# HKU-MedAI/WSI-HGNN

Hardware: AMD Instinct MI355X
Metric: edges/s fwd+bwd HEATNet4, 10k-node/6-rel synth graph, 1->8 MI355X (higher is better)
Workload: dtype f32 (fp16x3 emulation: 2-way fp16 split scaled per row (Y = XW^T, dX) or per column (dW), 3 products - bf16x6 for small launches; fp32-class error)

## Files before the change

### include/wsi_hgnn.h

```cpp
#ifndef WSI_HGNN_H
#define WSI_HGNN_H

#include <stdint.h>

#ifdef __cplusplus
extern "C" {
#endif

#define WSI_OK        0
#define WSI_EINVAL  (-22)
#define WSI_ENOSYS  (-38)
#define WSI_EFAULT  (-14)
#define WSI_ENOMEM  (-12)

#define WSI_ABI_VERSION 26

int         wsi_abi_version(void);
const char* wsi_last_error(void);

typedef struct wsi_context wsi_context_t;
int  wsi_context_create(wsi_context_t** out);
void wsi_context_destroy(wsi_context_t* ctx);

#define WSI_ATTN_XCD_CONTIGUOUS 1
// ... 198 lines not shown
int wsi_bag_slot_fill(const int64_t* bag_desc, int32_t num_bags, const int32_t* sel, float* rows, int64_t ld, int32_t feats,
                      int64_t num_rows, int32_t* row_seg, int32_t filler_seg,
                      const int32_t* small_src, int32_t* small_dst, int32_t small_words, void* stream);

typedef struct wsi_adam_tensor { float* p; const float* g; float* m; float* v; int64_t n; } wsi_adam_tensor_t;
int wsi_adam_step(const wsi_adam_tensor_t* tensors, int32_t count, double lr, double beta1, double beta2, double eps,
                  double weight_decay, int64_t step, void* stream);

#define WSI_OPTIM_SGD      0
#define WSI_OPTIM_ADAGRAD  1
#define WSI_OPTIM_ADADELTA 2
#define WSI_OPTIM_ADAM     3
#define WSI_OPTIM_FIRST    1
typedef struct wsi_optim_tensor {
    float* p; const float* g; float* s0; float* s1;
    float* step; int32_t* ticket; int64_t n; int32_t flags;
} wsi_optim_tensor_t;
typedef struct wsi_optim_hyper {
    double lr, weight_decay, momentum, dampening, nesterov, lr_decay, eps, rho, beta1, beta2, host_step;
} wsi_optim_hyper_t;
int wsi_optim_step(int32_t rule, const wsi_optim_tensor_t* tensors, int32_t count, const wsi_optim_hyper_t* hyper, void* stream);

int wsi_cross_entropy(const float* logits, const int64_t* labels, int32_t B, int32_t C, float* loss, float* dlogits, int32_t* bad_label, void* stream);

int wsi_segment_dot_diff(const float* g, int64_t ldg, const float* a, int64_t lda, const float* b, int64_t ldb,
                         int32_t D, const int32_t* chunk_row, int32_t num_chunks,
                         const int32_t* seg_chunk, int32_t num_segs,
                         float* partial, float* out, void* stream);

int wsi_gate_grad(const float* g, int64_t ldg, const float* a, int64_t lda, const float* b, int64_t ldb,
                  int32_t D, const int32_t* chunk_row, int32_t num_chunks, const int32_t* seg_chunk, int32_t num_segs,
                  const int32_t* seg_gate, const float* skip, int32_t n_gates, float* partial, float* g_skip, void* stream);

int wsi_pool_factors(const float* x, int64_t ldx, int32_t D, const float* w, int64_t ldw, int32_t T, int32_t H, int32_t Bg,
                     const int32_t* chunk_row, int32_t num_chunks, const int32_t* seg_chunk,
                     float* partial, float* hp, float* csum, float* x_mean, void* stream);
int wsi_pool_tmean(const float* tpart, int32_t T, int32_t S, int32_t D, int32_t H, const float* csum, const float* const* bv,
                   const float* scale, float* t_mean, void* stream);
int wsi_pool_bwd_prep(const float* g_pool, int32_t S, int32_t D, int32_t op, const float* counts, const float* z_mean, const float* h_mean,
                      const int32_t* seg_gate, const float* skip, int32_t n_gates, const int32_t* type_gate, int32_t T,
                      float* g_row, float* g_sum, float* g_skip, float* omg, void* stream);
int wsi_pool_bwd_bias(const float* gt_seg, int32_t T, int32_t S, int32_t D, int32_t H, const float* const* bv, const float* csum,
                      float* beta, float* gbv, void* stream);

int wsi_plan_assemble(const int64_t* desc, int32_t nsegs, int32_t total_blocks, void* stream);
int wsi_slot_fill(const int64_t* desc, int32_t nsegs, int32_t total_blocks, void* stream);

int wsi_layernorm_fwd(const float* x, int64_t ldx, int32_t n, int32_t D, float eps,
                      const float* gamma, const float* beta, const int32_t* row_param,
                      float* y, int64_t ldy, float* stats, void* stream);
int wsi_layernorm_bwd(const float* gy, int64_t ldgy, const float* x, int64_t ldx, int32_t n, int32_t D,
                      const float* gamma, const int32_t* row_param, const float* stats,
                      float* gx, int64_t ldgx, float* xhat_gy, int64_t ldp, void* stream);
int wsi_gelu_fwd(const float* x, float* y, int64_t n, void* stream);
int wsi_gelu_bwd(const float* x, const float* gy, float* gx, int64_t n, void* stream);
int wsi_spmm_sum(const float* x, int64_t ldx, int32_t n_out, int32_t D,
                 const int32_t* ptr, const int32_t* idx, const float* edge_w, const float* iscale, const float* oscale,
                 const float* bias, int32_t relu, const float* relu_ref, int64_t ldref,
                 float* out, int64_t ldo, void* stream);
int wsi_sddmm_dot(const float* g, int64_t ldg, const float* x, int64_t ldx, int32_t n, int32_t D,
                  const int32_t* rowptr, const int32_t* src, const float* iscale, const float* oscale,
                  const float* relu_ref, int64_t ldref, float* g_w, void* stream);

int wsi_row_sqnorm(const float* x, int64_t ldx, int32_t n, int32_t F, float* out, void* stream);
int wsi_knn_select(const float* dots, int64_t ldd, const float* sqnorm, int32_t row0, int32_t rows, int32_t N,
                   int32_t kc, int32_t* cand, void* stream);
// ... 166 lines not shown
```

### wsi-hgnn_amd/csrc/common.h

```cpp
#pragma once
#include <hip/hip_runtime.h>
#include <stdint.h>
#include <stdio.h>
#include <stdarg.h>
#include <stdlib.h>

#include "../../include/wsi_hgnn.h"

namespace wsi {

void set_error(const char* fmt, ...);

#ifdef WSI_ABLATE
inline const char* knob(const char* name) { return getenv(name); }
#else
constexpr const char* knob(const char*) { return nullptr; }
#endif

inline int check_launch(const char* what) {
    hipError_t e = hipGetLastError();
    if (e != hipSuccess) {
        set_error("%s: %s", what, hipGetErrorString(e));
        return WSI_EFAULT;
    }
    return WSI_OK;
}

template <int CTRL>
__device__ __forceinline__ float dpp_mov(float x) {
    return __int_as_float(__builtin_amdgcn_update_dpp(0, __float_as_int(x), CTRL, 0xf, 0xf, true));
}

template <int LPH>
__device__ __forceinline__ float group_sum(float x) {
    if (LPH >= 2) x += dpp_mov<0xB1>(x);
    if (LPH >= 4) x += dpp_mov<0x4E>(x);
    if (LPH >= 8) x += dpp_mov<0x141>(x);
    if (LPH >= 16) x += dpp_mov<0x140>(x);
    if (LPH >= 32) x += __shfl_xor(x, 16);
    if (LPH >= 64) x += __shfl_xor(x, 32);
    return x;
}

__device__ __forceinline__ float wave_sum(float x) { return group_sum<64>(x); }

template <int V>
__device__ __forceinline__ void load_vec(float (&r)[V], const float* __restrict__ p) {
    if constexpr (V % 4 == 0) {
#pragma unroll
        for (int i = 0; i < V / 4; ++i) {
            const float4 t = reinterpret_cast<const float4*>(p)[i];
            r[4 * i + 0] = t.x; r[4 * i + 1] = t.y; r[4 * i + 2] = t.z; r[4 * i + 3] = t.w;
        }
    } else if constexpr (V == 2) {
        const float2 t = *reinterpret_cast<const float2*>(p);
        r[0] = t.x; r[1] = t.y;
    } else {
#pragma unroll
        for (int i = 0; i < V; ++i) r[i] = p[i];
    }
}

template <int V>
__device__ __forceinline__ void store_vec(float* __restrict__ p, const float (&r)[V]) {
    if constexpr (V % 4 == 0) {
#pragma unroll
        for (int i = 0; i < V / 4; ++i)
            reinterpret_cast<float4*>(p)[i] = make_float4(r[4 * i], r[4 * i + 1], r[4 * i + 2], r[4 * i + 3]);
// ... 10 lines not shown
```

### wsi-hgnn_amd/csrc/heat_attn.hip

```cpp
#include "common.h"
#include <math.h>
#include <stdlib.h>
#include <mutex>
#include <type_traits>
#include <new>

namespace wsi {

struct AttnGraph {
    const int32_t* node_seg;
    const int32_t* rowptr;
    const int32_t* src;
    const float* sim;
    const int32_t* order;
    int32_t num_nodes;
    int32_t heavy_n;
    int32_t pass;
    int32_t heavy_deg;
    int32_t xcd;
    uint32_t* absmax;
    const float* score_in;
    const int32_t* gt_row;
};

// ... 318 lines not shown
                const float bj = beta[((int64_t)tau * S + (b * segs_per_type + gb)) * H + hh];
                gtab[(int64_t)ra * J + j] = acc_a[q] + bj;
                if (two) gtab[(int64_t)rbb * J + j] = acc_b[q] + bj;
            }
        }
    }
}

__global__ __launch_bounds__(256) void heat_attn_bwd_p1_flat_kernel(
    const int32_t* __restrict__ src, const int32_t* __restrict__ edge_seg, const int32_t* __restrict__ seg_dst,
    const int32_t* __restrict__ row_seg, int32_t segs_per_type, int32_t n_types, const float* __restrict__ inv_rd,
    const float* __restrict__ gtab, const float* __restrict__ lse, int64_t EH, int32_t H, const float* score_in, float* score_a, float* __restrict__ ga) {
    const int64_t o = (int64_t)blockIdx.x * 256 + threadIdx.x;
    if (o >= EH) return;
    const int64_t e = o / H;
    const int hh = (int)(o - e * H);
    const int s = edge_seg[e];
    const int w = seg_dst[s];
    const int b = row_seg[w] / segs_per_type;
    score_a[o] = expf(score_in[o] - lse[(int64_t)s * H + hh]);
    ga[o] = gtab[((int64_t)src[e] * n_types + b) * H + hh] * inv_rd[w];
}

__global__ __launch_bounds__(256) void heat_pool_coeff_kernel(
    const float* __restrict__ score, const float* __restrict__ lse, const int32_t* __restrict__ edge_seg,
    const int32_t* __restrict__ colptr, const int32_t* __restrict__ csc_eid, const int32_t* __restrict__ csc_dst,
    const float* __restrict__ inv_rd, const int32_t* __restrict__ row_seg, int32_t segs_per_type, int32_t n_types, int32_t H,
    int32_t num_src, float* __restrict__ ctab) {
    const int64_t idx = (int64_t)blockIdx.x * 256 + threadIdx.x;
    if (idx >= (int64_t)num_src * H) return;
    const int u = (int)(idx / H), h = (int)(idx - (int64_t)u * H);
    float cb[kPoolTypes];
#pragma unroll
    for (int b = 0; b < kPoolTypes; ++b) cb[b] = 0.f;
    const int j0 = colptr[u], j1 = colptr[u + 1];
    for (int j = j0; j < j1; ++j) {
        const int e = csc_eid[j], w = csc_dst[j];
        const float a = expf(score[(int64_t)e * H + h] - lse[(int64_t)edge_seg[e] * H + h]) * inv_rd[w];
        const int bin = row_seg[w] / segs_per_type;
#pragma unroll
        for (int b = 0; b < kPoolTypes; ++b) cb[b] += (bin == b) ? a : 0.f;
    }
#pragma unroll
    for (int b = 0; b < kPoolTypes; ++b)
        if (b < n_types) ctab[((int64_t)u * n_types + b) * H + h] = cb[b];
}

template <int V, int LPH, int U, bool COOP = false>
__global__ __launch_bounds__(kBlock) void heat_attn_bwd_p2_kernel(
    AttnTables tb, AttnGraph g, const float* __restrict__ e_weight, const float* __restrict__ e_bias,
    float inv_sqrt_dk, const float* __restrict__ a, const float* __restrict__ ga,
    float* __restrict__ gsc, float* __restrict__ gea, float* __restrict__ gq, int64_t ldgq) {
    constexpr int H = 64 / LPH;
    __shared__ float sm_acc[COOP ? kWavesPerBlock * 64 * V : 1];
    int lane;
    const int w = wave_uniform_node<COOP>(g, lane);
    if (w < 0) return;
    const int part = COOP ? (int)(threadIdx.x >> 6) : 0;
    constexpr int ESTEP = COOP ? kWavesPerBlock * U : U;
// ... 946 lines not shown
```

### wsi-hgnn_amd/csrc/loss.hip

```cpp
#include "common.h"
#include <math.h>

namespace wsi {

constexpr int64_t CE_IGNORE_INDEX = -100;
__global__ __launch_bounds__(256) void cross_entropy_kernel(const float* __restrict__ logits, const int64_t* __restrict__ labels, int B, int C,
                                                            float* __restrict__ loss, float* __restrict__ dlogits, int* __restrict__ bad) {
    __shared__ float part[256];
    __shared__ int cnt[256];
    __shared__ int any_bad;
    if (threadIdx.x == 0) any_bad = 0;
    int valid = 0;
    for (int b = threadIdx.x; b < B; b += 256) {
        const int64_t y = labels[b];
        valid += (y >= 0 && y < C) ? 1 : 0;
    }
    cnt[threadIdx.x] = valid;
    __syncthreads();
    for (int o = 128; o > 0; o >>= 1) {
        if ((int)threadIdx.x < o) cnt[threadIdx.x] += cnt[threadIdx.x + o];
        __syncthreads();
    }
    const int nvalid = cnt[0];
    const float invB = nvalid > 0 ? 1.f / (float)nvalid : 0.f;
    float acc = 0.f;
    for (int b = threadIdx.x; b < B; b += 256) {
        const float* row = logits + (int64_t)b * C;
        const int64_t y = labels[b];
        if (y < 0 || y >= C) {
            if (y != CE_IGNORE_INDEX) { any_bad = 1; if (bad) *bad = 1; }
            for (int c = 0; c < C; ++c) dlogits[(int64_t)b * C + c] = 0.f;
            continue;
        }
        float mx = -INFINITY;
// ... 1 lines not shown
        float den = 0.f;
        for (int c = 0; c < C; ++c) den += expf(row[c] - mx);
        acc += (logf(den) + mx) - row[y];
        const float inv = 1.f / den;
        for (int c = 0; c < C; ++c) dlogits[(int64_t)b * C + c] = (expf(row[c] - mx) * inv - (c == y ? 1.f : 0.f)) * invB;
    }
    part[threadIdx.x] = acc;
    __syncthreads();
    for (int o = 128; o > 0; o >>= 1) {
        if ((int)threadIdx.x < o) part[threadIdx.x] += part[threadIdx.x + o];
        __syncthreads();
    }
    if (threadIdx.x == 0) *loss = any_bad ? NAN : part[0] / (float)nvalid;
}

}

using namespace wsi;

extern "C" int wsi_cross_entropy(const float* logits, const int64_t* labels, int32_t B, int32_t C, float* loss, float* dlogits, int32_t* bad_label,
                                 void* stream) {
    if (B <= 0 || C <= 0 || (int64_t)B * C > 65536) { set_error("cross_entropy: unsupported shape %d x %d", B, C); return WSI_ENOSYS; }
    if (!logits || !labels || !loss || !dlogits) { set_error("cross_entropy: null pointer"); return WSI_EINVAL; }
    hipLaunchKernelGGL(cross_entropy_kernel, dim3(1), dim3(256), 0, (hipStream_t)stream, logits, labels, (int)B, (int)C, loss, dlogits, (int*)bad_label);
    return check_launch("cross_entropy");
}
```

### wsi-hgnn_amd/csrc/pooled.hip

```cpp
#include "common.h"
#include <math.h>

namespace wsi {

constexpr int POOL_MAX_TYPES = 16;
struct PtrList { const float* p[POOL_MAX_TYPES]; };

__global__ __launch_bounds__(256) void pool_tmean_kernel(const float* __restrict__ tpart, int tau0, int nt, int T, int S, int D, int H,
                                                         const float* __restrict__ csum, const PtrList bv, const float* __restrict__ scale,
                                                         int accumulate, int finish, float* __restrict__ t_mean) {
    const int s = blockIdx.x, c = blockIdx.y * 256 + threadIdx.x;
    if (c >= D) return;
    const int hh = c / (D / H);
    float acc = accumulate ? t_mean[(int64_t)s * D + c] : 0.f;
    for (int i = 0; i < nt; ++i) {
        const int tau = tau0 + i;
        acc += tpart[((int64_t)tau * S + s) * D + c];
        if (bv.p[i]) acc = fmaf(csum[((int64_t)tau * S + s) * H + hh], bv.p[i][c], acc);
    }
    if (finish && scale) acc *= scale[s];
    t_mean[(int64_t)s * D + c] = acc;
}

__global__ __launch_bounds__(256) void pool_bwd_prep_kernel(const float* __restrict__ g_pool, int S, int D, int mean, const float* __restrict__ counts,
// ... 4 lines not shown
                                                            float* __restrict__ omg) {
    extern __shared__ float dots[];
    const int lane = threadIdx.x & 63, wave = threadIdx.x >> 6;
    for (int s = wave; s < S; s += 4) {
        const float cnt = counts[s];
        const float fr = mean ? (cnt > 0.f ? 1.f / cnt : 0.f) : 1.f;
        const float fs = mean ? (cnt > 0.f ? 1.f : 0.f) : cnt;
        float acc = 0.f;
        for (int c = lane; c < D; c += 64) {
            const int64_t i = (int64_t)s * D + c;
            const float g = g_pool[i];
            const float gs = g * fs;
            g_row[i] = g * fr;
            g_sum[i] = gs;
            acc = fmaf(gs, z_mean[i] - h_mean[i], acc);
        }
        acc = wave_sum(acc);
        if (lane == 0) dots[s] = acc;
    }
    __syncthreads();
    for (int gt = threadIdx.x; gt < n_gates; gt += 256) {
        float acc = 0.f;
        for (int s = 0; s < S; ++s) acc += (seg_gate[s] == gt) ? dots[s] : 0.f;
        g_skip[gt] = acc * (1.f - 1.f / (1.f + expf(-skip[gt])));
    }
    for (int i = threadIdx.x; i < T; i += 256) {
        const int gt = type_gate[i];
        omg[i] = gt >= 0 ? 1.f - 1.f / (1.f + expf(-skip[gt])) : 1.f;
    }
}

__global__ __launch_bounds__(256) void pool_bwd_bias_kernel(const float* __restrict__ gt_seg, int tau0, int nt, int S, int D, int H, const PtrList bv,
                                                            const float* __restrict__ csum, float* __restrict__ beta, float* __restrict__ gbv) {
    const int dk = D / H;
    int blk = blockIdx.x;
    if (beta) {
        if (blk < nt * S) {
            const int i = blk / S, s = blk - i * S, tau = tau0 + i;
            const int lane = threadIdx.x & 63, wave = threadIdx.x >> 6;
            for (int hh = wave; hh < H; hh += 4) {
                float acc = 0.f;
                if (bv.p[i])
                    for (int c = lane; c < dk; c += 64) acc = fmaf(gt_seg[(int64_t)s * D + hh * dk + c], bv.p[i][hh * dk + c], acc);
                acc = wave_sum(acc);
                if (lane == 0) beta[((int64_t)tau * S + s) * H + hh] = acc;
            }
// ... 22 lines not shown
    hipStream_t st = (hipStream_t)stream;
    for (int t0 = 0; t0 < T; t0 += POOL_MAX_TYPES) {
        const int nt = (T - t0 < POOL_MAX_TYPES) ? T - t0 : POOL_MAX_TYPES;
        PtrList L;
        for (int i = 0; i < POOL_MAX_TYPES; ++i) L.p[i] = (i < nt) ? bv[t0 + i] : nullptr;
        hipLaunchKernelGGL(pool_tmean_kernel, dim3(S, (D + 255) / 256), dim3(256), 0, st, tpart, t0, nt, (int)T, (int)S, (int)D, (int)H, csum, L, scale,
                           t0 > 0 ? 1 : 0, t0 + nt >= T ? 1 : 0, t_mean);
    }
    return check_launch("pool_tmean");
}

extern "C" int wsi_pool_bwd_prep(const float* g_pool, int32_t S, int32_t D, int32_t op, const float* counts, const float* z_mean, const float* h_mean,
                                 const int32_t* seg_gate, const float* skip, int32_t n_gates, const int32_t* type_gate, int32_t T,
                                 float* g_row, float* g_sum, float* g_skip, float* omg, void* stream) {
    if (S <= 0 || S > 8192 || D <= 0 || n_gates <= 0 || T <= 0 || (op != WSI_RED_SUM && op != WSI_RED_MEAN)) { set_error("pool_bwd_prep: bad argument"); return WSI_EINVAL; }
    if (!g_pool || !counts || !z_mean || !h_mean || !seg_gate || !skip || !type_gate || !g_row || !g_sum || !g_skip || !omg) {
        set_error("pool_bwd_prep: null pointer"); return WSI_EINVAL;
    }
    hipLaunchKernelGGL(pool_bwd_prep_kernel, dim3(1), dim3(256), (size_t)S * sizeof(float), (hipStream_t)stream, g_pool, (int)S, (int)D,
                       op == WSI_RED_MEAN ? 1 : 0, counts, z_mean, h_mean, seg_gate, skip, (int)n_gates, type_gate, (int)T, g_row, g_sum, g_skip, omg);
    return check_launch("pool_bwd_prep");
}

extern "C" int wsi_pool_bwd_bias(const float* gt_seg, int32_t T, int32_t S, int32_t D, int32_t H, const float* const* bv, const float* csum,
                                 float* beta, float* gbv, void* stream) {
    if (T <= 0 || S <= 0 || D <= 0 || H <= 0 || D % H) { set_error("pool_bwd_bias: bad argument"); return WSI_EINVAL; }
    if (!gt_seg || (beta && !bv) || (gbv && !csum)) { set_error("pool_bwd_bias: null pointer"); return WSI_EINVAL; }
    if (!beta && !gbv) return WSI_OK;
    hipStream_t st = (hipStream_t)stream;
    const int tiles = (D + 255) / 256;
    for (int t0 = 0; t0 < T; t0 += POOL_MAX_TYPES) {
        const int nt = (T - t0 < POOL_MAX_TYPES) ? T - t0 : POOL_MAX_TYPES;
        PtrList L;
        for (int i = 0; i < POOL_MAX_TYPES; ++i) L.p[i] = (beta && i < nt) ? bv[t0 + i] : nullptr;
        const int blocks = (beta ? nt * S : 0) + (gbv ? nt * tiles : 0);
        hipLaunchKernelGGL(pool_bwd_bias_kernel, dim3(blocks), dim3(256), 0, st, gt_seg, t0, nt, (int)S, (int)D, (int)H, L, csum, beta, gbv);
    }
    return check_launch("pool_bwd_bias");
}
```

### wsi-hgnn_amd/csrc/segment.hip

```cpp
#include "common.h"
#include <math.h>

namespace wsi {

constexpr int SEG_THREADS = 256;

template <int OP>
__global__ __launch_bounds__(SEG_THREADS) void seg_stage1(const float* __restrict__ x, int64_t ldx, int32_t D, bool vec,
                                                           const int32_t* __restrict__ chunk_row,
                                                           float* __restrict__ partial, int32_t* __restrict__ partial_arg) {
    const int c = blockIdx.x;
    const int lane = threadIdx.x & 63, wave = threadIdx.x >> 6;
    const int col = blockIdx.y * 256 + lane * 4;
    const int r0 = chunk_row[c], r1 = chunk_row[c + 1];
    float a[4];
    int arg[4];
#pragma unroll
    for (int i = 0; i < 4; ++i) { a[i] = (OP == WSI_RED_MAX) ? -INFINITY : 0.f; arg[i] = -1; }
    if (col < D) {
        for (int r = r0 + wave; r < r1; r += 4) {
            const float* p = x + (int64_t)r * ldx + col;
            float v[4];
            if (vec && col + 3 < D) {
                const float4 t = *reinterpret_cast<const float4*>(p);
// ... 40 lines not shown
    const int col = blockIdx.y * SEG_THREADS + threadIdx.x;
    if (col >= D) return;
    const int c0 = seg_chunk[s], c1 = seg_chunk[s + 1];
    float acc = (OP == WSI_RED_MAX) ? -INFINITY : 0.f;
    int arg = -1;
    for (int c = c0; c < c1; ++c) {
        const float v = partial[(int64_t)c * D + col];
        if (OP == WSI_RED_MAX) {
            if (v > acc) { acc = v; arg = partial_arg[(int64_t)c * D + col]; }
        } else acc += v;
    }
    if (OP == WSI_RED_MEAN) {
        const int cnt = (c1 > c0) ? chunk_row[c1] - chunk_row[c0] : 0;
        acc = acc / (float)(cnt > 0 ? cnt : 1);
    }
    if (OP == WSI_RED_MAX) {
        if (arg < 0) acc = 0.f;
        argmax[(int64_t)s * D + col] = arg;
    }
    out[(int64_t)s * ldo + col] = acc;
}

constexpr int WSUM_J = 16;
__global__ __launch_bounds__(SEG_THREADS) void seg_wsum_stage1(const float* __restrict__ x, int64_t ldx, int32_t D, bool vec,
                                                                const float* __restrict__ w, int64_t ldw, int32_t JW, int32_t J,
                                                                const int32_t* __restrict__ chunk_row, float* __restrict__ partial,
                                                                float* __restrict__ wpartial) {
    const int c = blockIdx.x;
    const int lane = threadIdx.x & 63;
    const int wave = __builtin_amdgcn_readfirstlane((int)(threadIdx.x >> 6));
    const int col = blockIdx.y * 256 + lane * 4;
    const int jb = blockIdx.z * WSUM_J;
    const int nj = min(WSUM_J, J - jb);
    const int r0 = chunk_row[c], r1 = chunk_row[c + 1];
    float a[WSUM_J][4];
    float ws[WSUM_J];
#pragma unroll
    for (int j = 0; j < WSUM_J; ++j) {
        ws[j] = 0.f;
#pragma unroll
        for (int i = 0; i < 4; ++i) a[j][i] = 0.f;
    }
    if (col < D) {
        for (int r = r0 + wave; r < r1; r += 4) {
            const float* p = x + (int64_t)r * ldx + col;
            float v[4];
            if (vec && col + 3 < D) {
                const float4 t = *reinterpret_cast<const float4*>(p);
                v[0] = t.x; v[1] = t.y; v[2] = t.z; v[3] = t.w;
            } else {
#pragma unroll
                for (int i = 0; i < 4; ++i) v[i] = (col + i < D) ? p[i] : 0.f;
            }
            const float* wr = w + (int64_t)r * ldw + jb;
#pragma unroll
            for (int j = 0; j < WSUM_J; ++j) {
                const float wj = (jb + j < JW) ? wr[j] : ((j < nj) ? 1.f : 0.f);
                ws[j] += wj;
#pragma unroll
                for (int i = 0; i < 4; ++i) a[j][i] = fmaf(wj, v[i], a[j][i]);
            }
        }
    }
    if (wpartial && blockIdx.y == 0) {
        __shared__ float shw[4][WSUM_J];
        if (lane == 0) {
#pragma unroll
// ... 136 lines not shown

__global__ __launch_bounds__(256) void gate_grad_stage2(const float* __restrict__ partial, int32_t ncoltiles, const int32_t* __restrict__ seg_chunk,
                                                        int32_t num_segs, const int32_t* __restrict__ seg_gate, const float* __restrict__ skip,
                                                        int32_t n_gates, float* __restrict__ g_skip) {
    extern __shared__ float dots[];
    const int lane = threadIdx.x & 63, wave = threadIdx.x >> 6;
    for (int s = wave; s < num_segs; s += 4) {
        const int64_t p0 = (int64_t)seg_chunk[s] * ncoltiles, p1 = (int64_t)seg_chunk[s + 1] * ncoltiles;
        float acc = 0.f;
        for (int64_t i = p0 + lane; i < p1; i += 64) acc += partial[i];
        acc = wave_sum(acc);
        if (lane == 0) dots[s] = acc;
    }
    __syncthreads();
    for (int gt = threadIdx.x; gt < n_gates; gt += 256) {
        float acc = 0.f;
        for (int s = 0; s < num_segs; ++s) acc += (seg_gate[s] == gt) ? dots[s] : 0.f;
        g_skip[gt] = acc * (1.f - 1.f / (1.f + expf(-skip[gt])));
    }
}

static inline bool vec_ok(const void* p, int64_t ld) { return ((reinterpret_cast<uintptr_t>(p) & 15) == 0) && (ld % 4 == 0); }

}

using namespace wsi;

extern "C" int wsi_segment_reduce_fwd(const float* x, int64_t ldx, int32_t D, int32_t op,
                                      const int32_t* chunk_row, int32_t num_chunks,
                                      const int32_t* seg_chunk, int32_t num_segs,
                                      float* partial, float* out, int64_t ldo, int32_t* argmax, void* stream) {
    if (D <= 0 || num_chunks < 0 || num_segs < 0 || op < 0 || op > 2) { set_error("segment_reduce_fwd: bad argument"); return WSI_EINVAL; }
    if (num_segs == 0) return WSI_OK;
    if (!chunk_row || !seg_chunk || !out || (num_chunks > 0 && (!x || !partial))) { set_error("segment_reduce_fwd: null pointer"); return WSI_EINVAL; }
    if (op == WSI_RED_MAX && !argmax) { set_error("segment_reduce_fwd: max needs argmax"); return WSI_EINVAL; }
    hipStream_t st = (hipStream_t)stream;
    const bool vec = vec_ok(x, ldx);
    int32_t* parg = reinterpret_cast<int32_t*>(partial + (int64_t)num_chunks * D);
    const dim3 g1(num_chunks, (D + 255) / 256), g2(num_segs, (D + SEG_THREADS - 1) / SEG_THREADS);
    if (op == WSI_RED_SUM) {
        if (num_chunks) hipLaunchKernelGGL(seg_stage1<WSI_RED_SUM>, g1, dim3(SEG_THREADS), 0, st, x, ldx, D, vec, chunk_row, partial, (int32_t*)nullptr);
        hipLaunchKernelGGL(seg_stage2<WSI_RED_SUM>, g2, dim3(SEG_THREADS), 0, st, (const float*)partial, (const int32_t*)nullptr, D, chunk_row, seg_chunk, out, ldo, (int32_t*)nullptr);
    } else if (op == WSI_RED_MEAN) {
        if (num_chunks) hipLaunchKernelGGL(seg_stage1<WSI_RED_SUM>, g1, dim3(SEG_THREADS), 0, st, x, ldx, D, vec, chunk_row, partial, (int32_t*)nullptr);
        hipLaunchKernelGGL(seg_stage2<WSI_RED_MEAN>, g2, dim3(SEG_THREADS), 0, st, (const float*)partial, (const int32_t*)nullptr, D, chunk_row, seg_chunk, out, ldo, (int32_t*)nullptr);
    } else {
// ... 27 lines not shown
                                    float* partial, float* out, void* stream) {
    if (D <= 0 || num_chunks < 0 || num_segs < 0) { set_error("segment_dot_diff: bad argument"); return WSI_EINVAL; }
    if (num_segs == 0) return WSI_OK;
    if (!chunk_row || !seg_chunk || !out || (num_chunks > 0 && (!g || !a || !b || !partial))) { set_error("segment_dot_diff: null pointer"); return WSI_EINVAL; }
    hipStream_t st = (hipStream_t)stream;
    const int nct = (D + 255) / 256;
    const bool vec = vec_ok(g, ldg) && vec_ok(a, lda) && vec_ok(b, ldb);
    if (num_chunks) hipLaunchKernelGGL(seg_dot_stage1, dim3(num_chunks, nct), dim3(SEG_THREADS), 0, st, g, ldg, a, lda, b, ldb, D, vec, chunk_row, partial);
    hipLaunchKernelGGL(seg_dot_stage2, dim3(num_segs), dim3(64), 0, st, (const float*)partial, nct, seg_chunk, out);
    return check_launch("segment_dot_diff");
}

extern "C" int wsi_segment_weighted_sums(const float* x, int64_t ldx, int32_t D, const float* w, int64_t ldw, int32_t J,
                                         const int32_t* chunk_row, int32_t num_chunks, const int32_t* seg_chunk, int32_t num_segs,
                                         float* partial, float* out, void* stream) {
    if (D <= 0 || J <= 0 || J > 1024 || num_chunks < 0 || num_segs < 0) { set_error("segment_weighted_sums: bad argument"); return WSI_EINVAL; }
    if (num_segs == 0) return WSI_OK;
    if (!chunk_row || !seg_chunk || !out || (num_chunks > 0 && (!x || !w || !partial))) { set_error("segment_weighted_sums: null pointer"); return WSI_EINVAL; }
    if ((int64_t)J * D > INT32_MAX) { set_error("segment_weighted_sums: J * D too large"); return WSI_EINVAL; }
    hipStream_t st = (hipStream_t)stream;
    const bool vec = vec_ok(x, ldx);
    const int32_t JD = J * D;
    const dim3 g1(num_chunks, (D + 255) / 256, (J + WSUM_J - 1) / WSUM_J), g2(num_segs, (JD + SEG_THREADS - 1) / SEG_THREADS);
    if (num_chunks) hipLaunchKernelGGL(seg_wsum_stage1, g1, dim3(SEG_THREADS), 0, st, x, ldx, D, vec, w, ldw, J, J, chunk_row, partial, (float*)nullptr);
    hipLaunchKernelGGL(seg_stage2<WSI_RED_SUM>, g2, dim3(SEG_THREADS), 0, st, (const float*)partial, (const int32_t*)nullptr, JD, chunk_row, seg_chunk,
                       out, (int64_t)JD, (int32_t*)nullptr);
    return check_launch("segment_weighted_sums");
}

extern "C" int wsi_pool_factors(const float* x, int64_t ldx, int32_t D, const float* w, int64_t ldw, int32_t T, int32_t H, int32_t Bg,
                                const int32_t* chunk_row, int32_t num_chunks, const int32_t* seg_chunk,
                                float* partial, float* hp, float* csum, float* x_mean, void* stream) {
    if (D <= 0 || T <= 0 || H <= 0 || Bg <= 0 || num_chunks < 0 || (int64_t)T * H > 1024) { set_error("pool_factors: bad argument"); return WSI_EINVAL; }
    if (!chunk_row || !seg_chunk || !hp || !csum || (num_chunks > 0 && (!x || !w || !partial))) { set_error("pool_factors: null pointer"); return WSI_EINVAL; }
    const int32_t J = T * H, JT = J + (x_mean ? 1 : 0);
    if ((int64_t)JT * D > INT32_MAX) { set_error("pool_factors: T * H * D too large"); return WSI_EINVAL; }
    hipStream_t st = (hipStream_t)stream;
    float* wpartial = partial + (int64_t)num_chunks * JT * D;
    const dim3 g1(num_chunks, (D + 255) / 256, (JT + WSUM_J - 1) / WSUM_J);
    const dim3 g2(T * Bg, (uint32_t)(((int64_t)JT * D + SEG_THREADS - 1) / SEG_THREADS) + 1);
    if (num_chunks) hipLaunchKernelGGL(seg_wsum_stage1, g1, dim3(SEG_THREADS), 0, st, x, ldx, D, vec_ok(x, ldx), w, ldw, J, JT, chunk_row, partial, wpartial);
    hipLaunchKernelGGL(pool_factors_stage2, g2, dim3(SEG_THREADS), 0, st, (const float*)partial, (const float*)wpartial, D, T, H, Bg, JT, chunk_row, seg_chunk,
                       hp, csum, x_mean);
    return check_launch("pool_factors");
}

extern "C" int wsi_gate_grad(const float* g, int64_t ldg, const float* a, int64_t lda, const float* b, int64_t ldb,
                             int32_t D, const int32_t* chunk_row, int32_t num_chunks, const int32_t* seg_chunk, int32_t num_segs,
                             const int32_t* seg_gate, const float* skip, int32_t n_gates, float* partial, float* g_skip, void* stream) {
    if (D <= 0 || num_chunks < 0 || num_segs < 0 || n_gates <= 0 || num_segs > 8192) { set_error("gate_grad: bad argument"); return WSI_EINVAL; }
    if (!chunk_row || !seg_chunk || !seg_gate || !skip || !g_skip || (num_chunks > 0 && (!g || !a || !b || !partial))) { set_error("gate_grad: null pointer"); return WSI_EINVAL; }
    hipStream_t st = (hipStream_t)stream;
    const int nct = (D + 255) / 256;
    const bool vec = vec_ok(g, ldg) && vec_ok(a, lda) && vec_ok(b, ldb);
    if (num_chunks) hipLaunchKernelGGL(seg_dot_stage1, dim3(num_chunks, nct), dim3(SEG_THREADS), 0, st, g, ldg, a, lda, b, ldb, D, vec, chunk_row, partial);
    hipLaunchKernelGGL(gate_grad_stage2, dim3(1), dim3(256), (size_t)(num_segs > 0 ? num_segs : 1) * sizeof(float), st, (const float*)partial, nct, seg_chunk,
                       num_segs, seg_gate, skip, n_gates, g_skip);
    return check_launch("gate_grad");
}
```

### wsi-hgnn_amd/ops.py

```python
from __future__ import annotations

import array
import ctypes
import contextlib
from typing import List, Optional, Sequence, Tuple

import torch

from . import _native as N
from .graph import GraphPlan, SegmentTable, host_to_device



_TIMING = {"on": False, "records": []}


def enable_kernel_timing(on: bool) -> None:
    _TIMING["on"] = bool(on)
    _TIMING["records"] = []


class _Timed:
    def __init__(self, name: str, flops: float = 0.0, mfma_flops: float = 0.0):
        self.name, self.flops, self.mfma_flops = name, flops, mfma_flops
# ... 379 lines not shown
            N.check(lib.wsi_gemm_grouped(op, epilogue, prec, arr, len(chunk), N.ptr(ws), ws_bytes, N.stream()), "wsi_gemm_grouped")
    return wrote


_GROUP_FIELDS = [f[0] for f in N.GemmGroup._fields_]
_GROUP_INDEX = {name: i for i, name in enumerate(_GROUP_FIELDS)}
_GROUP_DEFAULT = tuple(1.0 if name == "drop_scale" else (None if N.GemmGroup._fields_[i][1] is ctypes.c_void_p else 0) for i, name in enumerate(_GROUP_FIELDS))


def _group_array(chunk):
    index, default = _GROUP_INDEX, _GROUP_DEFAULT
    rows = []
    for g in chunk:
        vals = list(default)
        for k, v in g.items():
            i = index.get(k)
            if i is not None:
                vals[i] = v
        rows.append(N.GemmGroup(*vals))
    return (N.GemmGroup * len(rows))(*rows)


_SMALL_PAIR = {"enabled": True}


def _gemm_small_pair(dx_groups: Sequence[dict], dx_epilogue: int, dw_groups: Sequence[dict], dw_epilogue: int, device) -> bool:
    dx_groups = [g for g in dx_groups if g["M"] > 0 and g["N"] > 0]
    dw_groups = [g for g in dw_groups if g["M"] > 0 and g["N"] > 0]
    if (not _SMALL_PAIR["enabled"] or not dx_groups or not dw_groups or len(dx_groups) + len(dw_groups) > 16
            or any(g["M"] > 32 or g.get("c_absmax") or g.get("b_chunk") for g in dx_groups) or any(g["K"] > 32 or g.get("c_absmax") for g in dw_groups)):
        return False
    flops = sum(2.0 * g["M"] * g["N"] * g["K"] for g in list(dx_groups) + list(dw_groups))
    with _Timed("gemm", flops, flops), _Timed("gemm_small_pair", flops, flops):
        N.check(N.load().wsi_gemm_small_pair(_group_array(dx_groups), len(dx_groups), dx_epilogue, _group_array(dw_groups), len(dw_groups), dw_epilogue,
                                             N.stream()), "wsi_gemm_small_pair")
    return True


_BACKGROUND = {"enabled": True, "min_flop": 3.0e10, "queued": [], "pending": [], "armed": False, "blocked": False,
               "launches": 0, "task": -1, "written": set()}


def set_background_weight_gradients(on: bool) -> None:
    _BACKGROUND["enabled"] = bool(on)


# ... 1083 lines not shown
        ctx.save_for_backward(h, kqv, t, out, score, lse, skip, ew, eb, sim_csr, *(() if (drop_mask is None or counter is not None) else (drop_mask,)), *params)
        return out

    @staticmethod
    def backward(ctx, g_out):
        lib = N.load()
        hctx, H, T = ctx.hctx, ctx.H, ctx.T
        bc = None
        if ctx.pool is not None:
            h, kqv, t_mean, h_mean, z_mean, score, lse, skip, ew, eb, sim_csr, *params = ctx.saved_tensors
            fwd_factors = None
            if ctx.no_v:
                fwd_factors, params = params[:3], params[3:]
            t = out = None
            prp, pop = ctx.pool
            n_rows, D_ = h.shape
            pre = None
            segs_p = prp.segments_of(hctx.rows)
            if prp.num_segs <= 8192 and segs_p is not None:
                seg_gate, type_gate = _gate_tables(hctx, skip, segs_p, prp.num_segs)
                g_pool = g_out.contiguous()
                g_row, g_sum = torch.empty_like(g_pool), torch.empty_like(g_pool)
                pre = (torch.empty_like(skip), torch.empty(T, dtype=torch.float32, device=h.device))
                N.check(lib.wsi_pool_bwd_prep(N.ptr(g_pool), prp.num_segs, D_, pop, N.ptr(prp.counts()), N.ptr(z_mean), N.ptr(h_mean), N.ptr(seg_gate),
                                              N.ptr(skip), skip.shape[0], N.ptr(type_gate), T, N.ptr(g_row), N.ptr(g_sum), N.ptr(pre[0]), N.ptr(pre[1]),
                                              N.stream()), "wsi_pool_bwd_prep")
                bc = SegmentBroadcast.from_parts(prp, g_row, g_sum, z_mean)
            else:
                bc = SegmentBroadcast.from_pooled_gradient(g_out.contiguous(), prp, pop, z_mean)
            collapse = ctx.no_v or _value_collapse_applies(hctx, prp, n_rows, D_, H)
            if collapse:
                g_out = None
            else:
                g_out = torch.empty((n_rows, D_), dtype=torch.float32, device=h.device)
                N.check(lib.wsi_segment_reduce_bwd(N.ptr(bc.g_row), D_, D_, N.WSI_RED_SUM, N.ptr(prp.chunk_row), N.ptr(prp.chunk_seg),
                                                   prp.num_chunks, N.ptr(prp.seg_chunk), prp.num_segs, None,
                                                   N.ptr(g_out), D_, N.stream()), "wsi_segment_reduce_bwd")
        else:
            h, kqv, t, out, score, lse, skip, ew, eb, sim_csr, *params = ctx.saved_tensors
            t_mean = h_mean = None
            collapse = False
            fwd_factors = None
            pre = None
            g_out = g_out.contiguous()
        g_y = g_out
        if ctx.has_mask and getattr(ctx, "counter", None) is not None:
            g_y = dropout_apply(g_out, ctx.counter)
        elif ctx.has_mask:
            g_y = g_out * params[0]
# ... 233 lines not shown
                grads[8 * tau + 6] = gbv[tau]
                for hh in range(H):
                    wgroups.append(dict(A=N.ptr(gt_seg, hh * dk * 4), lda=D, B=N.ptr(hp, (hh * T + tau) * D * 4), ldb=H * T * D,
                                        C=N.ptr(gw, hh * dk * D * 4), ldc=D, M=dk, N=D, K=S))
            _gemm(N.WSI_GEMM_TN, 0, wgroups, dev)
        if gh_max is not None and chunked:
            attach_row_scales(g_h, gh_max)
        if gh_cols is not None and gh_wrote and chunked:
            attach_col_stats(g_h, gh_cols)
        if early_gate is not None:
            torch.cuda.current_stream(dev).wait_event(early_gate[1])
        return (g_h, None, None, g_skip, g_e[0:1].view(1, 1), g_e[1:2], None, None, None, *grads)


def heat_layer_fused(h, hctx, H, skip, e_weight, e_bias, params, drop_mask=None, pool=None, background_dw=False):
    if pool is not None:
        pool = (pool[0], {"sum": N.WSI_RED_SUM, "mean": N.WSI_RED_MEAN}[pool[1]])
    return _HeatLayerFused.apply(h, hctx, H, skip, e_weight, e_bias, drop_mask, pool, background_dw, *params)


class _CrossEntropy(torch.autograd.Function):

    @staticmethod
    def forward(ctx, logits, labels, bad):
        N.require_cuda(logits, labels)
        logits = logits.contiguous()
        labels = labels.contiguous()
        if labels.dtype != torch.int64 or logits.dim() != 2 or labels.shape != logits.shape[:1]:
            raise ValueError("cross_entropy: logits [B, C] fp32 and int64 labels [B]")
        B, C = logits.shape
        out = torch.empty(1 + B * C, dtype=torch.float32, device=logits.device)
        N.check(N.load().wsi_cross_entropy(N.ptr(logits), N.ptr(labels), B, C, N.ptr(out), N.ptr(out, 4), N.ptr(bad), N.stream()), "wsi_cross_entropy")
        ctx.save_for_backward(out)
        ctx.shape = (B, C)
        return out[0]

    @staticmethod
    def backward(ctx, g):
        (out,) = ctx.saved_tensors
        return out[1:].view(ctx.shape) * g, None, None


def cross_entropy(logits: torch.Tensor, labels: torch.Tensor) -> torch.Tensor:
    bad = torch.zeros(1, dtype=torch.int32, device=logits.device)
    loss = _CrossEntropy.apply(logits, labels, bad)
    loss._wsi_bad_label = bad
    return loss


class _RelationAttention(torch.autograd.Function):

    @staticmethod
    def forward(ctx, q, kv, e_weight, e_bias, plan: GraphPlan, sim_csr, D: int, H: int):
        N.require_cuda(q, kv)
        lib = N.load()
        q = q.contiguous()
        kv = kv.contiguous()
        n, E, S = plan.num_nodes, plan.num_edges, plan.num_segs
        dev = q.device
        t = torch.empty((n, D), dtype=torch.float32, device=dev)
        score = torch.empty((max(E, 1), H), dtype=torch.float32, device=dev)
        lse = torch.empty((max(S, 1), H), dtype=torch.float32, device=dev)
        ew, eb = e_weight.reshape(-1), e_bias.reshape(-1)
        with _Timed("heat_attn"):
            N.check(lib.wsi_heat_attn_fwd(
                N.ptr(q), q.stride(0), N.ptr(kv, 0), kv.stride(0), N.ptr(kv, D * 4), kv.stride(0), n, D, H,
                N.ptr(plan.node_seg), N.ptr(plan.rowptr), N.ptr(plan.src), N.ptr(sim_csr), N.ptr(plan.order_dst), plan.num_heavy, _attn_flags(plan),
                N.ptr(ew), N.ptr(eb), N.ptr(t), D, N.ptr(score), N.ptr(lse), None, N.context(), N.stream()), "wsi_heat_attn_fwd")
# ... 1226 lines not shown
```

Before: 111.1 million.

## Spread pool backward prep across blocks, batch gathers, and drop CE zero-fill

```diff
diff --git a/include/wsi_hgnn.h b/include/wsi_hgnn.h
--- a/include/wsi_hgnn.h
+++ b/include/wsi_hgnn.h
@@ -244,6 +244,7 @@
 int wsi_optim_step(int32_t rule, const wsi_optim_tensor_t* tensors, int32_t count, const wsi_optim_hyper_t* hyper, void* stream);
 
 int wsi_cross_entropy(const float* logits, const int64_t* labels, int32_t B, int32_t C, float* loss, float* dlogits, int32_t* bad_label, void* stream);
+int wsi_cross_entropy_self(const float* logits, const int64_t* labels, int32_t B, int32_t C, float* loss, float* dlogits, int32_t* bad_label, void* stream);
 
 int wsi_segment_dot_diff(const float* g, int64_t ldg, const float* a, int64_t lda, const float* b, int64_t ldb,
                          int32_t D, const int32_t* chunk_row, int32_t num_chunks,
@@ -264,6 +265,9 @@
                       float* g_row, float* g_sum, float* g_skip, float* omg, void* stream);
 int wsi_pool_bwd_bias(const float* gt_seg, int32_t T, int32_t S, int32_t D, int32_t H, const float* const* bv, const float* csum,
                       float* beta, float* gbv, void* stream);
+int wsi_pool_bwd_prep_spread(const float* g_pool, int32_t S, int32_t D, int32_t op, const float* counts, const float* z_mean, const float* h_mean,
+                             const int32_t* seg_gate, const float* skip, int32_t n_gates, const int32_t* type_gate, int32_t T,
+                             float* g_row, float* g_sum, float* g_skip, float* omg, float* dots, int32_t* ticket, void* stream);
 
 int wsi_plan_assemble(const int64_t* desc, int32_t nsegs, int32_t total_blocks, void* stream);
 int wsi_slot_fill(const int64_t* desc, int32_t nsegs, int32_t total_blocks, void* stream);
diff --git a/wsi-hgnn_amd/csrc/common.h b/wsi-hgnn_amd/csrc/common.h
--- a/wsi-hgnn_amd/csrc/common.h
+++ b/wsi-hgnn_amd/csrc/common.h
@@ -44,6 +44,24 @@
 
 __device__ __forceinline__ float wave_sum(float x) { return group_sum<64>(x); }
 
+__device__ __forceinline__ void publish(float* p, float v) { __hip_atomic_store(p, v, __ATOMIC_RELAXED, __HIP_MEMORY_SCOPE_AGENT); }
+
+__device__ __forceinline__ bool arrive_last(int32_t* ticket, int blocks, int* flag) {
+    asm volatile("s_waitcnt vmcnt(0)" ::: "memory");
+    __syncthreads();
+    if (threadIdx.x == 0) {
+        const int last = __hip_atomic_fetch_add(ticket, 1, __ATOMIC_RELAXED, __HIP_MEMORY_SCOPE_AGENT) == blocks - 1;
+        if (last) {
+            __hip_atomic_exchange(ticket, 0, __ATOMIC_RELAXED, __HIP_MEMORY_SCOPE_AGENT);
+            __builtin_amdgcn_fence(__ATOMIC_ACQUIRE, "agent");
+            asm volatile("s_waitcnt vmcnt(0)" ::: "memory");
+        }
+        *flag = last;
+    }
+    __syncthreads();
+    return *flag != 0;
+}
+
 template <int V>
 __device__ __forceinline__ void load_vec(float (&r)[V], const float* __restrict__ p) {
     if constexpr (V % 4 == 0) {
diff --git a/wsi-hgnn_amd/csrc/heat_attn.hip b/wsi-hgnn_amd/csrc/heat_attn.hip
--- a/wsi-hgnn_amd/csrc/heat_attn.hip
+++ b/wsi-hgnn_amd/csrc/heat_attn.hip
@@ -364,6 +364,28 @@
     ga[o] = gtab[((int64_t)src[e] * n_types + b) * H + hh] * inv_rd[w];
 }
 
+template <int NB>
+__device__ __forceinline__ void pool_coeff_edges(int j, int h, int H, int segs_per_type, const float* __restrict__ score, const float* __restrict__ lse,
+                                                 const int32_t* __restrict__ edge_seg, const int32_t* __restrict__ csc_eid,
+                                                 const int32_t* __restrict__ csc_dst, const float* __restrict__ inv_rd,
+                                                 const int32_t* __restrict__ row_seg, float (&cb)[kPoolTypes]) {
+    int e[NB], w[NB], sg[NB], rs[NB];
+    float sc[NB], ls[NB], ir[NB];
+#pragma unroll
+    for (int i = 0; i < NB; ++i) { e[i] = csc_eid[j + i]; w[i] = csc_dst[j + i]; }
+#pragma unroll
+    for (int i = 0; i < NB; ++i) { sg[i] = edge_seg[e[i]]; sc[i] = score[(int64_t)e[i] * H + h]; ir[i] = inv_rd[w[i]]; rs[i] = row_seg[w[i]]; }
+#pragma unroll
+    for (int i = 0; i < NB; ++i) ls[i] = lse[(int64_t)sg[i] * H + h];
+#pragma unroll
+    for (int i = 0; i < NB; ++i) {
+        const float a = expf(sc[i] - ls[i]) * ir[i];
+        const int bin = rs[i] / segs_per_type;
+#pragma unroll
+        for (int b = 0; b < kPoolTypes; ++b) cb[b] += (bin == b) ? a : 0.f;
+    }
+}
+
 __global__ __launch_bounds__(256) void heat_pool_coeff_kernel(
     const float* __restrict__ score, const float* __restrict__ lse, const int32_t* __restrict__ edge_seg,
     const int32_t* __restrict__ colptr, const int32_t* __restrict__ csc_eid, const int32_t* __restrict__ csc_dst,
@@ -376,7 +398,10 @@
 #pragma unroll
     for (int b = 0; b < kPoolTypes; ++b) cb[b] = 0.f;
     const int j0 = colptr[u], j1 = colptr[u + 1];
-    for (int j = j0; j < j1; ++j) {
+    int j = j0;
+    for (; j + 8 <= j1; j += 8) pool_coeff_edges<8>(j, h, H, segs_per_type, score, lse, edge_seg, csc_eid, csc_dst, inv_rd, row_seg, cb);
+    for (; j + 4 <= j1; j += 4) pool_coeff_edges<4>(j, h, H, segs_per_type, score, lse, edge_seg, csc_eid, csc_dst, inv_rd, row_seg, cb);
+    for (; j < j1; ++j) {
         const int e = csc_eid[j], w = csc_dst[j];
         const float a = expf(score[(int64_t)e * H + h] - lse[(int64_t)edge_seg[e] * H + h]) * inv_rd[w];
         const int bin = row_seg[w] / segs_per_type;
diff --git a/wsi-hgnn_amd/csrc/loss.hip b/wsi-hgnn_amd/csrc/loss.hip
--- a/wsi-hgnn_amd/csrc/loss.hip
+++ b/wsi-hgnn_amd/csrc/loss.hip
@@ -5,11 +5,14 @@
 
 constexpr int64_t CE_IGNORE_INDEX = -100;
 __global__ __launch_bounds__(256) void cross_entropy_kernel(const float* __restrict__ logits, const int64_t* __restrict__ labels, int B, int C,
-                                                            float* __restrict__ loss, float* __restrict__ dlogits, int* __restrict__ bad) {
+                                                            float* __restrict__ loss, float* __restrict__ dlogits, int* __restrict__ bad, int clear_bad) {
     __shared__ float part[256];
     __shared__ int cnt[256];
     __shared__ int any_bad;
-    if (threadIdx.x == 0) any_bad = 0;
+    if (threadIdx.x == 0) {
+        any_bad = 0;
+        if (clear_bad && bad) *bad = 0;
+    }
     int valid = 0;
     for (int b = threadIdx.x; b < B; b += 256) {
         const int64_t y = labels[b];
@@ -57,6 +60,14 @@
                                  void* stream) {
     if (B <= 0 || C <= 0 || (int64_t)B * C > 65536) { set_error("cross_entropy: unsupported shape %d x %d", B, C); return WSI_ENOSYS; }
     if (!logits || !labels || !loss || !dlogits) { set_error("cross_entropy: null pointer"); return WSI_EINVAL; }
-    hipLaunchKernelGGL(cross_entropy_kernel, dim3(1), dim3(256), 0, (hipStream_t)stream, logits, labels, (int)B, (int)C, loss, dlogits, (int*)bad_label);
+    hipLaunchKernelGGL(cross_entropy_kernel, dim3(1), dim3(256), 0, (hipStream_t)stream, logits, labels, (int)B, (int)C, loss, dlogits, (int*)bad_label, 0);
     return check_launch("cross_entropy");
 }
+
+extern "C" int wsi_cross_entropy_self(const float* logits, const int64_t* labels, int32_t B, int32_t C, float* loss, float* dlogits, int32_t* bad_label,
+                                      void* stream) {
+    if (B <= 0 || C <= 0 || (int64_t)B * C > 65536) { set_error("cross_entropy: unsupported shape %d x %d", B, C); return WSI_ENOSYS; }
+    if (!logits || !labels || !loss || !dlogits) { set_error("cross_entropy: null pointer"); return WSI_EINVAL; }
+    hipLaunchKernelGGL(cross_entropy_kernel, dim3(1), dim3(256), 0, (hipStream_t)stream, logits, labels, (int)B, (int)C, loss, dlogits, (int*)bad_label, 1);
+    return check_launch("cross_entropy");
+}
diff --git a/wsi-hgnn_amd/csrc/pooled.hip b/wsi-hgnn_amd/csrc/pooled.hip
--- a/wsi-hgnn_amd/csrc/pooled.hip
+++ b/wsi-hgnn_amd/csrc/pooled.hip
@@ -50,6 +50,43 @@
     for (int gt = threadIdx.x; gt < n_gates; gt += 256) {
         float acc = 0.f;
         for (int s = 0; s < S; ++s) acc += (seg_gate[s] == gt) ? dots[s] : 0.f;
+        g_skip[gt] = acc * (1.f - 1.f / (1.f + expf(-skip[gt])));
+    }
+    for (int i = threadIdx.x; i < T; i += 256) {
+        const int gt = type_gate[i];
+        omg[i] = gt >= 0 ? 1.f - 1.f / (1.f + expf(-skip[gt])) : 1.f;
+    }
+}
+
+__global__ __launch_bounds__(256) void pool_bwd_prep_spread_kernel(const float* __restrict__ g_pool, int S, int D, int mean, const float* __restrict__ counts,
+                                                                   const float* __restrict__ z_mean, const float* __restrict__ h_mean,
+                                                                   const int32_t* __restrict__ seg_gate, const float* __restrict__ skip, int n_gates,
+                                                                   const int32_t* __restrict__ type_gate, int T,
+                                                                   float* __restrict__ g_row, float* __restrict__ g_sum, float* g_skip,
+                                                                   float* omg, float* dots, int32_t* ticket) {
+    __shared__ int last;
+    const int lane = threadIdx.x & 63, wave = threadIdx.x >> 6;
+    const int s = blockIdx.x * 4 + wave;
+    if (s < S) {
+        const float cnt = counts[s];
+        const float fr = mean ? (cnt > 0.f ? 1.f / cnt : 0.f) : 1.f;
+        const float fs = mean ? (cnt > 0.f ? 1.f : 0.f) : cnt;
+        float acc = 0.f;
+        for (int c = lane; c < D; c += 64) {
+            const int64_t i = (int64_t)s * D + c;
+            const float g = g_pool[i];
+            const float gs = g * fs;
+            g_row[i] = g * fr;
+            g_sum[i] = gs;
+            acc = fmaf(gs, z_mean[i] - h_mean[i], acc);
+        }
+        acc = wave_sum(acc);
+        if (lane == 0) publish(dots + s, acc);
+    }
+    if (!arrive_last(ticket, (int)gridDim.x, &last)) return;
+    for (int gt = threadIdx.x; gt < n_gates; gt += 256) {
+        float acc = 0.f;
+        for (int q = 0; q < S; ++q) acc += (seg_gate[q] == gt) ? dots[q] : 0.f;
         g_skip[gt] = acc * (1.f - 1.f / (1.f + expf(-skip[gt])));
     }
     for (int i = threadIdx.x; i < T; i += 256) {
@@ -118,6 +155,19 @@
     return check_launch("pool_bwd_prep");
 }
 
+extern "C" int wsi_pool_bwd_prep_spread(const float* g_pool, int32_t S, int32_t D, int32_t op, const float* counts, const float* z_mean, const float* h_mean,
+                                        const int32_t* seg_gate, const float* skip, int32_t n_gates, const int32_t* type_gate, int32_t T,
+                                        float* g_row, float* g_sum, float* g_skip, float* omg, float* dots, int32_t* ticket, void* stream) {
+    if (S <= 0 || S > 8192 || D <= 0 || n_gates <= 0 || T <= 0 || (op != WSI_RED_SUM && op != WSI_RED_MEAN)) { set_error("pool_bwd_prep_spread: bad argument"); return WSI_EINVAL; }
+    if (!g_pool || !counts || !z_mean || !h_mean || !seg_gate || !skip || !type_gate || !g_row || !g_sum || !g_skip || !omg || !dots || !ticket) {
+        set_error("pool_bwd_prep_spread: null pointer"); return WSI_EINVAL;
+    }
+    hipLaunchKernelGGL(pool_bwd_prep_spread_kernel, dim3((S + 3) / 4), dim3(256), 0, (hipStream_t)stream, g_pool, (int)S, (int)D,
+                       op == WSI_RED_MEAN ? 1 : 0, counts, z_mean, h_mean, seg_gate, skip, (int)n_gates, type_gate, (int)T, g_row, g_sum, g_skip, omg,
+                       dots, ticket);
+    return check_launch("pool_bwd_prep_spread");
+}
+
 extern "C" int wsi_pool_bwd_bias(const float* gt_seg, int32_t T, int32_t S, int32_t D, int32_t H, const float* const* bv, const float* csum,
                                  float* beta, float* gbv, void* stream) {
     if (T <= 0 || S <= 0 || D <= 0 || H <= 0 || D % H) { set_error("pool_bwd_bias: bad argument"); return WSI_EINVAL; }
diff --git a/wsi-hgnn_amd/csrc/segment.hip b/wsi-hgnn_amd/csrc/segment.hip
--- a/wsi-hgnn_amd/csrc/segment.hip
+++ b/wsi-hgnn_amd/csrc/segment.hip
@@ -86,6 +86,7 @@
 }
 
 constexpr int WSUM_J = 16;
+template <bool STREAM>
 __global__ __launch_bounds__(SEG_THREADS) void seg_wsum_stage1(const float* __restrict__ x, int64_t ldx, int32_t D, bool vec,
                                                                 const float* __restrict__ w, int64_t ldw, int32_t JW, int32_t J,
                                                                 const int32_t* __restrict__ chunk_row, float* __restrict__ partial,
@@ -106,7 +107,30 @@
         for (int i = 0; i < 4; ++i) a[j][i] = 0.f;
     }
     if (col < D) {
-        for (int r = r0 + wave; r < r1; r += 4) {
+        int r = r0 + wave;
+        if constexpr (STREAM) {
+            for (; r + 12 < r1; r += 16) {
+                float4 t[4];
+                float wl[4];
+#pragma unroll
+                for (int q = 0; q < 4; ++q) t[q] = *reinterpret_cast<const float4*>(x + (int64_t)(r + 4 * q) * ldx + col);
+#pragma unroll
+                for (int q = 0; q < 4; ++q)
+                    wl[q] = (jb + lane < JW && lane < WSUM_J) ? w[(int64_t)(r + 4 * q) * ldw + jb + lane] : ((lane < nj) ? 1.f : 0.f);
+#pragma unroll
+                for (int q = 0; q < 4; ++q) {
+                    const float v[4] = {t[q].x, t[q].y, t[q].z, t[q].w};
+#pragma unroll
+                    for (int j = 0; j < WSUM_J; ++j) {
+                        const float wj = __int_as_float(__builtin_amdgcn_readlane(__float_as_int(wl[q]), j));
+                        ws[j] += wj;
+#pragma unroll
+                        for (int i = 0; i < 4; ++i) a[j][i] = fmaf(wj, v[i], a[j][i]);
+                    }
+                }
+            }
+        }
+        for (; r < r1; r += 4) {
             const float* p = x + (int64_t)r * ldx + col;
             float v[4];
             if (vec && col + 3 < D) {
@@ -289,6 +313,12 @@
 
 static inline bool vec_ok(const void* p, int64_t ld) { return ((reinterpret_cast<uintptr_t>(p) & 15) == 0) && (ld % 4 == 0); }
 
+static void launch_wsum_stage1(dim3 grid, hipStream_t st, const float* x, int64_t ldx, int32_t D, bool vec, const float* w, int64_t ldw, int32_t JW,
+                               int32_t J, const int32_t* chunk_row, float* partial, float* wpartial) {
+    if (vec && D % 4 == 0) hipLaunchKernelGGL(seg_wsum_stage1<true>, grid, dim3(SEG_THREADS), 0, st, x, ldx, D, vec, w, ldw, JW, J, chunk_row, partial, wpartial);
+    else hipLaunchKernelGGL(seg_wsum_stage1<false>, grid, dim3(SEG_THREADS), 0, st, x, ldx, D, vec, w, ldw, JW, J, chunk_row, partial, wpartial);
+}
+
 }
 
 using namespace wsi;
@@ -362,7 +392,7 @@
     const bool vec = vec_ok(x, ldx);
     const int32_t JD = J * D;
     const dim3 g1(num_chunks, (D + 255) / 256, (J + WSUM_J - 1) / WSUM_J), g2(num_segs, (JD + SEG_THREADS - 1) / SEG_THREADS);
-    if (num_chunks) hipLaunchKernelGGL(seg_wsum_stage1, g1, dim3(SEG_THREADS), 0, st, x, ldx, D, vec, w, ldw, J, J, chunk_row, partial, (float*)nullptr);
+    if (num_chunks) launch_wsum_stage1(g1, st, x, ldx, D, vec, w, ldw, J, J, chunk_row, partial, nullptr);
     hipLaunchKernelGGL(seg_stage2<WSI_RED_SUM>, g2, dim3(SEG_THREADS), 0, st, (const float*)partial, (const int32_t*)nullptr, JD, chunk_row, seg_chunk,
                        out, (int64_t)JD, (int32_t*)nullptr);
     return check_launch("segment_weighted_sums");
@@ -379,7 +409,7 @@
     float* wpartial = partial + (int64_t)num_chunks * JT * D;
     const dim3 g1(num_chunks, (D + 255) / 256, (JT + WSUM_J - 1) / WSUM_J);
     const dim3 g2(T * Bg, (uint32_t)(((int64_t)JT * D + SEG_THREADS - 1) / SEG_THREADS) + 1);
-    if (num_chunks) hipLaunchKernelGGL(seg_wsum_stage1, g1, dim3(SEG_THREADS), 0, st, x, ldx, D, vec_ok(x, ldx), w, ldw, J, JT, chunk_row, partial, wpartial);
+    if (num_chunks) launch_wsum_stage1(g1, st, x, ldx, D, vec_ok(x, ldx), w, ldw, J, JT, chunk_row, partial, wpartial);
     hipLaunchKernelGGL(pool_factors_stage2, g2, dim3(SEG_THREADS), 0, st, (const float*)partial, (const float*)wpartial, D, T, H, Bg, JT, chunk_row, seg_chunk,
                        hp, csum, x_mean);
     return check_launch("pool_factors");
diff --git a/wsi-hgnn_amd/ops.py b/wsi-hgnn_amd/ops.py
--- a/wsi-hgnn_amd/ops.py
+++ b/wsi-hgnn_amd/ops.py
@@ -425,6 +425,21 @@
 
 
 _SMALL_PAIR = {"enabled": True}
+
+_SROW = {"on": True, "tickets": {}}
+TICKET_POOL_PREP = 0
+
+
+def set_srow_fusion(on: bool) -> None:
+    _SROW["on"] = bool(on)
+
+
+def _ticket(device, which: int) -> int:
+    key = (device.type, device.index if device.index is not None else torch.cuda.current_device())
+    t = _SROW["tickets"].get(key)
+    if t is None:
+        t = _SROW["tickets"][key] = torch.zeros(16 * 8, dtype=torch.int32, device=device)
+    return N.ptr(t, which * 64)
 
 
 def _gemm_small_pair(dx_groups: Sequence[dict], dx_epilogue: int, dw_groups: Sequence[dict], dw_epilogue: int, device) -> bool:
@@ -1554,9 +1569,16 @@
                 g_pool = g_out.contiguous()
                 g_row, g_sum = torch.empty_like(g_pool), torch.empty_like(g_pool)
                 pre = (torch.empty_like(skip), torch.empty(T, dtype=torch.float32, device=h.device))
-                N.check(lib.wsi_pool_bwd_prep(N.ptr(g_pool), prp.num_segs, D_, pop, N.ptr(prp.counts()), N.ptr(z_mean), N.ptr(h_mean), N.ptr(seg_gate),
-                                              N.ptr(skip), skip.shape[0], N.ptr(type_gate), T, N.ptr(g_row), N.ptr(g_sum), N.ptr(pre[0]), N.ptr(pre[1]),
-                                              N.stream()), "wsi_pool_bwd_prep")
+                if _SROW["on"]:
+                    dots = torch.empty(prp.num_segs, dtype=torch.float32, device=h.device)
+                    N.check(lib.wsi_pool_bwd_prep_spread(N.ptr(g_pool), prp.num_segs, D_, pop, N.ptr(prp.counts()), N.ptr(z_mean), N.ptr(h_mean),
+                                                         N.ptr(seg_gate), N.ptr(skip), skip.shape[0], N.ptr(type_gate), T, N.ptr(g_row), N.ptr(g_sum),
+                                                         N.ptr(pre[0]), N.ptr(pre[1]), N.ptr(dots), _ticket(h.device, TICKET_POOL_PREP), N.stream()),
+                            "wsi_pool_bwd_prep_spread")
+                else:
+                    N.check(lib.wsi_pool_bwd_prep(N.ptr(g_pool), prp.num_segs, D_, pop, N.ptr(prp.counts()), N.ptr(z_mean), N.ptr(h_mean), N.ptr(seg_gate),
+                                                  N.ptr(skip), skip.shape[0], N.ptr(type_gate), T, N.ptr(g_row), N.ptr(g_sum), N.ptr(pre[0]), N.ptr(pre[1]),
+                                                  N.stream()), "wsi_pool_bwd_prep")
                 bc = SegmentBroadcast.from_parts(prp, g_row, g_sum, z_mean)
             else:
                 bc = SegmentBroadcast.from_pooled_gradient(g_out.contiguous(), prp, pop, z_mean)
@@ -1836,7 +1858,7 @@
 class _CrossEntropy(torch.autograd.Function):
 
     @staticmethod
-    def forward(ctx, logits, labels, bad):
+    def forward(ctx, logits, labels, bad, self_clear=False):
         N.require_cuda(logits, labels)
         logits = logits.contiguous()
         labels = labels.contiguous()
@@ -1844,7 +1866,11 @@
             raise ValueError("cross_entropy: logits [B, C] fp32 and int64 labels [B]")
         B, C = logits.shape
         out = torch.empty(1 + B * C, dtype=torch.float32, device=logits.device)
-        N.check(N.load().wsi_cross_entropy(N.ptr(logits), N.ptr(labels), B, C, N.ptr(out), N.ptr(out, 4), N.ptr(bad), N.stream()), "wsi_cross_entropy")
+        if self_clear:
+            N.check(N.load().wsi_cross_entropy_self(N.ptr(logits), N.ptr(labels), B, C, N.ptr(out), N.ptr(out, 4), N.ptr(bad), N.stream()),
+                    "wsi_cross_entropy_self")
+        else:
+            N.check(N.load().wsi_cross_entropy(N.ptr(logits), N.ptr(labels), B, C, N.ptr(out), N.ptr(out, 4), N.ptr(bad), N.stream()), "wsi_cross_entropy")
         ctx.save_for_backward(out)
         ctx.shape = (B, C)
         return out[0]
@@ -1852,12 +1878,16 @@
     @staticmethod
     def backward(ctx, g):
         (out,) = ctx.saved_tensors
-        return out[1:].view(ctx.shape) * g, None, None
+        return out[1:].view(ctx.shape) * g, None, None, None
 
 
 def cross_entropy(logits: torch.Tensor, labels: torch.Tensor) -> torch.Tensor:
-    bad = torch.zeros(1, dtype=torch.int32, device=logits.device)
-    loss = _CrossEntropy.apply(logits, labels, bad)
+    if _SROW["on"]:
+        bad = torch.empty(1, dtype=torch.int32, device=logits.device)
+        loss = _CrossEntropy.apply(logits, labels, bad, True)
+    else:
+        bad = torch.zeros(1, dtype=torch.int32, device=logits.device)
+        loss = _CrossEntropy.apply(logits, labels, bad, False)
     loss._wsi_bad_label = bad
     return loss
 
```

Measured after the change: 108.7 million. -2.1%, worse.
